# OvO1111/JointImageGeneration

Hardware: AMD Instinct MI355X
Metric: sampled voxels/sec @50 DDIM steps, 128^3 mask + 512^2x256 CT (higher is better)
Workload: dtype bf16; 1 GPU; C5 full GuideGen volume per GPU: CCDM 128^3 K=14 250 steps -> LDM 256 slices x (cond-encode + 50 DDIM @4x64x64 + AE decode 512^2); volumes_per_gpu=1, ccdm_steps=250, ddim_steps=50, slices=256, parallelism=replicas x1 (one volume per GPU, no collective), weights=random-init (seed recipe)

## Files before the change

include/guidegen_hip.h:

```cpp
#ifndef GUIDEGEN_HIP_H
#define GUIDEGEN_HIP_H

#include <stdint.h>

#ifdef __cplusplus
extern "C" {
#endif

typedef enum {
    GG_OK = 0,
    GG_ERR_BAD_SHAPE = -1,
    GG_ERR_BAD_DTYPE = -2,
    GG_ERR_UNSUPPORTED = -3,
    GG_ERR_WORKSPACE_TOO_SMALL = -4,
    GG_ERR_HIP = -5
} gg_status;

typedef enum { GG_BF16 = 0, GG_F32 = 1 } gg_dtype;

const char *gg_last_error(void);
int gg_version(void);

typedef struct {
    int32_t N, D, H, W;
// ... 29 lines not shown
    int32_t epilogue_geglu;
    int32_t pro_c_logical;
    const int64_t *pro_acc1;
    const int64_t *pro_acc2;
    const float *pro_gamma;
    const float *pro_beta;
    float pro_eps;
    int32_t skip_C1, skip_C2;
    int32_t reserved_tail;
    const void *skip_src1;
    const void *skip_src2;
    const void *skip_weight;
    const int32_t *post_xt;
    int32_t *post_labels_out;
    const float *post_scalars;
    const float *post_E;
    uint64_t post_philox_seed;
    const int64_t *post_philox_offset_dev;
    void *post_onehot_out;
    int64_t post_onehot_stride;
    int32_t post_draw;
    int32_t reserved_tail2;
    const uint64_t *post_philox_seeds;
    int64_t post_rows_per_sample;
} gg_conv_desc;

int64_t gg_conv_packed_weight_bytes(int32_t Cout, int32_t Cin_pad, int32_t ntaps);
int gg_conv_pack_weight(const float *w_f32, int32_t Cout, int32_t Cin, int32_t Cin_pad, int32_t ntaps,
                        void *packed_bf16, void *stream);
int64_t gg_conv_workspace_bytes(const gg_conv_desc *desc);
int gg_conv_fuses_prologue(const gg_conv_desc *desc);
int gg_conv_fuses_posterior(const gg_conv_desc *desc);
int gg_conv_runs_halo_tile(const gg_conv_desc *desc);
int gg_conv_emits_stats(const gg_conv_desc *desc);
int gg_conv_prologue_from_acc(const gg_conv_desc *desc);
int gg_conv_fuses_skip(const gg_conv_desc *desc);
int gg_conv_fuses_ddim(const gg_conv_desc *desc);
int gg_conv_forward(const gg_conv_desc *desc, void *stream);

int64_t gg_groupnorm_workspace_bytes(int32_t N, int64_t S, int32_t C);
int gg_groupnorm_stats(const void *src1, int32_t C1, const void *src2, int32_t C2, int32_t N, int64_t S,
                       int32_t C_logical, const float *gamma, const float *beta, float eps,
                       float *scale_out, float *shift_out, void *workspace, int64_t workspace_bytes, void *stream);
int gg_groupnorm_apply(const void *src1, int32_t C1, const void *src2, int32_t C2, int32_t N, int64_t S,
                       const float *scale, const float *shift, int32_t act, void *out, void *stream);
int gg_groupnorm_fused_supported(int64_t S, int32_t C1, int32_t C2, int32_t C_logical);
int gg_groupnorm_fused(const void *src1, int32_t C1, const void *src2, int32_t C2, int32_t N, int64_t S, int32_t C_logical,
                       const float *gamma, const float *beta, float eps, int32_t act, void *out, void *stream);
int gg_groupnorm_apply_acc(const void *src1, int32_t C1, const int64_t *acc1, const void *src2, int32_t C2, const int64_t *acc2,
                           int32_t N, int64_t S, int32_t C_logical, const float *gamma, const float *beta, float eps,
                           int32_t act, void *out, void *stream);

int gg_groupnorm_scale_shift_acc(const int64_t *acc1, int32_t stripes1, int32_t C1, const int64_t *acc2, int32_t stripes2, int32_t C2,
                                 int32_t N, int64_t S, int32_t C_logical, const float *gamma, const float *beta, float eps,
                                 float *scale_out, float *shift_out, void *stream);

int gg_resample2x(const void *src, int32_t dtype, int32_t N, int32_t D, int32_t H, int32_t W, int32_t C_pad, int32_t C_logical,
                  int32_t resample_d, int32_t mode, const float *scale, const float *shift, int32_t act, void *dst, void *stream);
int gg_film_fold(float *scale, float *shift, int32_t coef_stride, int32_t N, int32_t C, const float *film, int64_t film_stride, void *stream);

typedef struct {
    int32_t N, heads, head_dim;
    int32_t Tq, Tkv;
    int64_t ldq, hsq, ldk, hsk, ldv, hsv, ldo, hso;
    float scale;
    int32_t reserved;
// ... 157 lines not shown
```

jointimagegeneration_amd/_lib.py:

```python
from __future__ import annotations

import ctypes as C
import os

_HERE = os.path.dirname(os.path.abspath(__file__))
LIB_PATH = os.path.join(_HERE, "csrc", "libguidegen_hip.so")

GG_BF16, GG_F32 = 0, 1

vp, i32, i64, u64, f32 = C.c_void_p, C.c_int32, C.c_int64, C.c_uint64, C.c_float


class ConvDesc(C.Structure):
    _fields_ = [
        ("N", i32), ("D", i32), ("H", i32), ("W", i32),
        ("C1", i32), ("C2", i32), ("Cout", i32), ("Cout_pad", i32),
        ("kd", i32), ("kh", i32), ("kw", i32), ("stride", i32), ("pad", i32), ("upsample", i32),
        ("Do", i32), ("Ho", i32), ("Wo", i32), ("out_dtype", i32), ("prologue_act", i32), ("path_hint", i32),
        ("src1", vp), ("src2", vp), ("weight", vp), ("bias", vp), ("bias_stride", i64),
        ("residual", vp), ("out", vp), ("gn_scale", vp), ("gn_shift", vp), ("workspace", vp), ("workspace_bytes", i64), ("reserved_ptr", vp), ("gn_acc", vp),
        ("ddim_x", vp), ("ddim_scalars", vp), ("ddim_pred_x0", vp), ("ddim_unet_in", vp), ("ddim_unet_in_stride", i64),
        ("epilogue_geglu", i32), ("pro_c_logical", i32), ("pro_acc1", vp), ("pro_acc2", vp), ("pro_gamma", vp), ("pro_beta", vp),
        ("pro_eps", f32), ("skip_C1", i32), ("skip_C2", i32), ("reserved_tail", i32), ("skip_src1", vp), ("skip_src2", vp), ("skip_weight", vp),
        ("post_xt", vp), ("post_labels_out", vp), ("post_scalars", vp), ("post_E", vp), ("post_philox_seed", C.c_uint64),
        ("post_philox_offset_dev", vp), ("post_onehot_out", vp), ("post_onehot_stride", i64), ("post_draw", i32), ("reserved_tail2", i32),
        ("post_philox_seeds", vp), ("post_rows_per_sample", i64),
    ]


class AttentionDesc(C.Structure):
    _fields_ = [
        ("N", i32), ("heads", i32), ("head_dim", i32), ("Tq", i32), ("Tkv", i32),
        ("ldq", i64), ("hsq", i64), ("ldk", i64), ("hsk", i64), ("ldv", i64), ("hsv", i64), ("ldo", i64), ("hso", i64),
        ("scale", f32), ("reserved", i32),
        ("q", vp), ("k", vp), ("v", vp), ("out", vp), ("workspace", vp), ("workspace_bytes", i64),
    ]


SIGNATURES = {
    "gg_last_error": (C.c_char_p, []),
    "gg_version": (C.c_int, []),
    "gg_conv_packed_weight_bytes": (i64, [i32, i32, i32]),
    "gg_conv_pack_weight": (C.c_int, [vp, i32, i32, i32, i32, vp, vp]),
    "gg_conv_forward": (C.c_int, [C.POINTER(ConvDesc), vp]),
    "gg_conv_workspace_bytes": (i64, [C.POINTER(ConvDesc)]),
    "gg_conv_fuses_prologue": (C.c_int, [C.POINTER(ConvDesc)]),
    "gg_conv_runs_halo_tile": (C.c_int, [C.POINTER(ConvDesc)]),
    "gg_conv_emits_stats": (C.c_int, [C.POINTER(ConvDesc)]),
    "gg_conv_prologue_from_acc": (C.c_int, [C.POINTER(ConvDesc)]),
    "gg_conv_fuses_skip": (C.c_int, [C.POINTER(ConvDesc)]),
    "gg_conv_fuses_ddim": (C.c_int, [C.POINTER(ConvDesc)]),
    "gg_conv_fuses_posterior": (C.c_int, [C.POINTER(ConvDesc)]),
    "gg_groupnorm_workspace_bytes": (i64, [i32, i64, i32]),
    "gg_groupnorm_stats": (C.c_int, [vp, i32, vp, i32, i32, i64, i32, vp, vp, f32, vp, vp, vp, i64, vp]),
    "gg_groupnorm_apply": (C.c_int, [vp, i32, vp, i32, i32, i64, vp, vp, i32, vp, vp]),
    "gg_groupnorm_apply_acc": (C.c_int, [vp, i32, vp, vp, i32, vp, i32, i64, i32, vp, vp, f32, i32, vp, vp]),
    "gg_groupnorm_fused_supported": (C.c_int, [i64, i32, i32, i32]),
    "gg_groupnorm_fused": (C.c_int, [vp, i32, vp, i32, i32, i64, i32, vp, vp, f32, i32, vp, vp]),
    "gg_groupnorm_scale_shift_acc": (C.c_int, [vp, i32, i32, vp, i32, i32, i32, i64, i32, vp, vp, f32, vp, vp, vp]),
    "gg_attention_forward": (C.c_int, [C.POINTER(AttentionDesc), vp]),
    "gg_attention_workspace_bytes": (i64, [C.POINTER(AttentionDesc)]),
    "gg_attention_plan": (C.c_int, [C.POINTER(AttentionDesc), C.POINTER(i32)]),
    "gg_attention_forward_kvlen": (C.c_int, [C.POINTER(AttentionDesc), vp, vp]),
    "gg_layernorm": (C.c_int, [vp, i64, i32, vp, vp, f32, vp, vp]),
    "gg_geglu": (C.c_int, [vp, i64, i32, vp, vp]),
    "gg_add": (C.c_int, [vp, vp, i64, vp, vp]),
    "gg_linear_f32": (C.c_int, [vp, i32, i32, vp, vp, i32, i32, vp, i64, vp]),
    "gg_timestep_embedding": (C.c_int, [vp, i32, i32, f32, vp, vp]),
    "gg_nchw_f32_to_cl_bf16": (C.c_int, [vp, i32, i32, i64, vp, i32, i32, i32, vp]),
    "gg_cl_to_nchw_f32": (C.c_int, [vp, i32, i32, i32, i64, i32, vp, vp]),
    "gg_ccdm_posterior_sample": (C.c_int, [vp, i32, i32, vp, vp, u64, vp, i32, vp, i32, i64, vp, vp, vp, i32, vp]),
    "gg_ccdm_posterior_sample_seeds": (C.c_int, [vp, i32, i32, vp, vp, vp, i64, vp, i32, vp, i32, i64, vp, vp, vp, i32, vp]),
    "gg_ccdm_draw_tape": (C.c_int, [u64, vp, i64, vp, i32, i64, vp, vp, vp, vp]),
    "gg_labels_to_onehot": (C.c_int, [vp, i64, i32, vp, i32, vp]),
    "gg_ddim_step": (C.c_int, [vp, vp, i32, vp, vp, i64, i32, vp, vp, i32, vp]),
    "gg_minmax_normalise": (C.c_int, [vp, i64, vp, vp, vp]),
    "gg_ddpm_step": (C.c_int, [vp, vp, i32, vp, vp, i64, i32, vp, i32, vp]),
    "gg_inpaint_blend": (C.c_int, [vp, vp, vp, i32, vp, vp, i64, i32, vp, i32, vp]),
    "gg_ddpm_step_x0": (C.c_int, [vp, vp, i32, vp, vp, i32, i64, i32, vp, vp, i32, vp]),
    "gg_log_rows": (C.c_int, [vp, i32, i32, i64, vp, vp]),
    "gg_vq_nearest": (C.c_int, [vp, i32, vp, i32, i32, i64, vp, vp, i32, vp]),
# ... 72 lines not shown
```

jointimagegeneration_amd/csrc/gg_conv.h:

```cpp
#pragma once
#include "gg_common.h"

struct ConvParams {
    int N, D, H, W, C1, C2, Cout, Cout_pad;
    int kd, kh, kw, stride, pad, upsample;
    int Do, Ho, Wo, out_dtype, prologue_act;
    int path_hint;
    int nchunk1, nchunk, ntaps;
    long long M;
    long long bias_stride;
    const bf16_t *src1, *src2, *weight, *residual;
    const float *bias, *gn_scale, *gn_shift;
    void *out;
    float *ws;
    int splitk;
    long long *gn_acc;
    float *ddim_x, *ddim_pred_x0;
    const float *ddim_scalars;
    bf16_t *ddim_unet_in;
    long long ddim_unet_in_stride;
    unsigned mg_osp, mg_ohw, mg_wo;
    int epi_geglu;
    const long long *pro_acc1, *pro_acc2;
    const float *pro_gamma, *pro_beta;
    float pro_eps;
    int pro_clog;
    const bf16_t *skip_src1, *skip_src2, *skip_weight;
    int skip_C1, skip_C2;
    const int *post_xt;
    int *post_labels_out;
    const float *post_scalars, *post_E;
    unsigned long long post_seed;
    const long long *post_offset_dev;
    bf16_t *post_onehot_out;
    long long post_onehot_stride;
    int post_draw;
    const unsigned long long *post_seeds;
    long long post_rows_per_sample;
};

#define GG_BOX_HINT_GENERIC 10
#define GG_BOX_HINT_SPEC_ONLY 11
#define GG_HALO_HINT_BOX512 1
#define GG_HALO_HINT_BOX256 4
#define GG_HALO_HINT_BOX1024 6
#define GG_HALO_HINT_TEAM 7
#define GG_HALO_HINT_NO_TEAM 8

#define GG_ACC_SUM_SCALE 268435456.0f
#define GG_ACC_SQ_SCALE 1048576.0f
#ifndef GG_ACC_STRIPES
#define GG_ACC_STRIPES 1
#endif
#define GG_ACC_STRIPES_HALO 32

__device__ __forceinline__ int swz64(int row, int chunk) { return chunk ^ ((row >> 1) & 2); }


__device__ __forceinline__ float gg_row16_sum(float x)
{
    x += __builtin_bit_cast(float, __builtin_amdgcn_mov_dpp(__builtin_bit_cast(int, x), 0xB1, 0xF, 0xF, true));
    x += __builtin_bit_cast(float, __builtin_amdgcn_mov_dpp(__builtin_bit_cast(int, x), 0x4E, 0xF, 0xF, true));
    x += __builtin_bit_cast(float, __builtin_amdgcn_mov_dpp(__builtin_bit_cast(int, x), 0x141, 0xF, 0xF, true));
    x += __builtin_bit_cast(float, __builtin_amdgcn_mov_dpp(__builtin_bit_cast(int, x), 0x140, 0xF, 0xF, true));
    return x;
}
```

jointimagegeneration_amd/csrc/gg_conv.hip:

```cpp
#include "gg_norm.h"
#include <stdlib.h>

template <int NT, int PF, int PRO>
__global__ __launch_bounds__(256) void conv_gather_kernel(const ConvParams p)
{
    constexpr int BM = 128;
    constexpr int XBYTES = BM * 64;
    constexpr int WBYTES = NT * 32 * 64;
    constexpr int STAGE = XBYTES + WBYTES;
    constexpr int WITER = (NT * 128 + 255) / 256;
    __shared__ __attribute__((aligned(16))) char smem[2 * STAGE];

    const int tid = threadIdx.x;
    const int lane = tid & 63;
    const int wave = tid >> 6;
    const long long m0 = (long long)blockIdx.x * BM;
    const int g0 = blockIdx.y * NT;

    const int xq = tid & 3;
    int bn[2], bd[2], bh[2], bw[2];
    bool rv[2];
    const bf16_t *rb1[2], *rb2[2];
    const unsigned osp = (unsigned)(p.Do * p.Ho * p.Wo);
    const unsigned ohw = (unsigned)(p.Ho * p.Wo);
// ... 182 lines not shown
                bf16x4 ob;
#pragma unroll
                for (int j = 0; j < 4; ++j) {
                    const float ge = 0.5f * g[j] * (1.0f + erff(g[j] * 0.70710678118654752f));
                    ob[j] = (bf16_t)((oc + j < inner) ? v[j] * ge : 0.f);
                }
                *reinterpret_cast<bf16x4 *>((bf16_t *)p.out + m * ostride + oc) = ob;
            }
        }
        return;
    }
    f32x4 bv[2][2 * NT];
    bf16x4 resv[2][2 * NT];
#pragma unroll
    for (int pt = 0; pt < 2; ++pt) {
        const long long m = m0 + wave * 32 + pt * 16 + fr;
        const long long mc = m < p.M ? m : p.M - 1;
        const int n = (int)((unsigned)mc / osp);
        const float *brow = p.bias ? p.bias + (long long)n * p.bias_stride : nullptr;
#pragma unroll
        for (int ct = 0; ct < 2 * NT; ++ct) {
            const int co = (g0 * 32) + ct * 16 + fq * 4;
            bv[pt][ct] = brow ? *reinterpret_cast<const f32x4 *>(brow + co) : f32x4{0.f, 0.f, 0.f, 0.f};
            if (p.residual) resv[pt][ct] = *reinterpret_cast<const bf16x4 *>(p.residual + mc * p.Cout_pad + co);
        }
    }
#pragma unroll
    for (int pt = 0; pt < 2; ++pt) {
        long long m = m0 + wave * 32 + pt * 16 + fr;
        if (m >= p.M) continue;
#pragma unroll
        for (int ct = 0; ct < 2 * NT; ++ct) {
            int co = (g0 * 32) + ct * 16 + fq * 4;
            f32x4 v = acc[pt][ct];
            if (p.bias) v += bv[pt][ct];
            long long o = m * p.Cout_pad + co;
            if (p.residual) {
                const bf16x4 r = resv[pt][ct];
#pragma unroll
                for (int j = 0; j < 4; ++j) v[j] += (float)r[j];
            }
#pragma unroll
            for (int j = 0; j < 4; ++j)
                if (co + j >= p.Cout) v[j] = 0.f;
            if (p.out_dtype == GG_F32) {
                *reinterpret_cast<f32x4 *>((float *)p.out + o) = v;
            } else {
                bf16x4 ob;
#pragma unroll
                for (int j = 0; j < 4; ++j) ob[j] = (bf16_t)v[j];
                *reinterpret_cast<bf16x4 *>((bf16_t *)p.out + o) = ob;
            }
        }
    }
}

template <int PRO>
__global__ __launch_bounds__(256) void conv_gather5_kernel(const ConvParams p)
{
    constexpr int BM = 64, CPS = 5;
    constexpr int XT = BM * 64, WT = 32 * 64;
    constexpr int STAGE = CPS * (XT + WT);
    constexpr int GNMAX = 2560;
    __shared__ __attribute__((aligned(16))) char smem[2 * STAGE + (PRO ? 2 * GNMAX * 4 : 0)];
    const int tid = threadIdx.x, lane = tid & 63;
    const int wave = __builtin_amdgcn_readfirstlane(tid >> 6);
    const int fr = lane & 15, fq = lane >> 4;
    const long long m0 = (long long)blockIdx.x * BM;
    const int g0 = blockIdx.y;
    float *gns = reinterpret_cast<float *>(smem + 2 * STAGE);

    const int xrow = tid >> 2, xq = tid & 3;
    const unsigned osp = (unsigned)(p.Do * p.Ho * p.Wo), ohw = (unsigned)(p.Ho * p.Wo);
    bool rv;
    int bd, bh, bw;
    const bf16_t *rb1, *rb2;
    {
        long long m = m0 + xrow;
        rv = m < p.M;
        unsigned mu = rv ? (unsigned)m : 0u;
        unsigned n = (unsigned)gg_fastdiv(mu, (int)osp, p.mg_osp), r = mu - n * osp;
        unsigned od = (unsigned)gg_fastdiv(r, (int)ohw, p.mg_ohw);
        r -= od * ohw;
        unsigned oh = (unsigned)gg_fastdiv(r, p.Wo, p.mg_wo), ow = r - oh * (unsigned)p.Wo;
// ... 405 lines not shown
    p.post_seeds = (const unsigned long long *)d->post_philox_seeds; p.post_rows_per_sample = d->post_rows_per_sample;
    p.mg_osp = gg_magic_u32(p.M, d->Do * d->Ho * d->Wo); p.mg_ohw = gg_magic_u32(p.M, d->Ho * d->Wo); p.mg_wo = gg_magic_u32(p.M, d->Wo);
}

static bool halo_try_dry(const ConvParams &p) { return gg_conv_halo_try(p, (hipStream_t)-1) == GG_OK; }
static bool box_try_dry(const ConvParams &p) { return gg_conv_box_try(p, (hipStream_t)-1) == GG_OK; }
static bool desc_channels_ok(const gg_conv_desc *d) { return d && d->C1 > 0 && d->C1 % 32 == 0 && d->C2 % 32 == 0 && d->Cout_pad % 32 == 0; }

static int take_splitk_workspace(const gg_conv_desc *d, ConvParams &p, int splitk)
{
    if (splitk > 1) {
        const long long need = (long long)splitk * p.M * p.Cout_pad * 4;
        if (!d->workspace || d->workspace_bytes < need)
            GG_FAIL(GG_ERR_WORKSPACE_TOO_SMALL, "conv: split-K needs %lld workspace bytes (gg_conv_workspace_bytes), got %lld", need, (long long)d->workspace_bytes);
        p.ws = (float *)d->workspace;
    }
    p.splitk = splitk;
    return GG_OK;
}

extern "C" int gg_conv_runs_halo_tile(const gg_conv_desc *d)
{
    if (!desc_channels_ok(d) || d->epilogue_geglu) return 0;
    ConvParams p;
    fill_params(d, p);
    return halo_try_dry(p) ? 1 : 0;
}

extern "C" int gg_conv_fuses_prologue(const gg_conv_desc *d)
{
    if (!desc_channels_ok(d) || d->epilogue_geglu) return 0;
    ConvParams p;
    fill_params(d, p);
    if (halo_try_dry(p)) return (GG_HALO_SEPARATE_NORM && d->path_hint == 0 && gg_conv_halo_prefers_separate_norm(p)) ? 0 : 1;
    if (box_try_dry(p)) return gg_conv_box_fuses_prologue(p) ? 1 : 0;
    return 0;
}

bool gg_conv_box_emits_stats(const ConvParams &p);
bool gg_conv_box_prologue_from_acc(const ConvParams &p);
bool gg_conv_halo_fuses_posterior(const ConvParams &p);

extern "C" int gg_conv_fuses_posterior(const gg_conv_desc *d)
{
    if (!desc_channels_ok(d) || d->epilogue_geglu || d->residual || d->out_dtype != GG_F32 || d->gn_acc ||
        d->ddim_x || d->skip_C1) return 0;
    ConvParams p;
    fill_params(d, p);
    return gg_conv_halo_fuses_posterior(p) ? 1 : 0;
}

extern "C" int gg_conv_prologue_from_acc(const gg_conv_desc *d)
{
    if (!desc_channels_ok(d) || d->epilogue_geglu || !d->prologue_act) return 0;
    if (d->pro_c_logical <= 0 || d->pro_c_logical % 32 || d->pro_c_logical > d->C1 + d->C2 || (d->C2 && d->pro_c_logical < d->C1)) return 0;
    ConvParams p;
    fill_params(d, p);
    if (halo_try_dry(p)) return 0;
    return box_try_dry(p) && gg_conv_box_prologue_from_acc(p) ? 1 : 0;
}

extern "C" int gg_conv_fuses_skip(const gg_conv_desc *d)
{
    if (!desc_channels_ok(d) || d->epilogue_geglu || d->skip_C1 <= 0 || d->skip_C1 % 32 || d->skip_C2 % 32 ||
        d->skip_C2 < 0 || d->residual || d->ddim_x)
        return 0;
    ConvParams p;
    fill_params(d, p);
    if (halo_try_dry(p)) return 0;
    return box_try_dry(p) ? 1 : 0;
}

extern "C" int gg_conv_fuses_ddim(const gg_conv_desc *d)
{
    if (!desc_channels_ok(d) || d->out_dtype != GG_F32 || d->Cout != 4 || d->residual) return 0;
    ConvParams p;
    fill_params(d, p);
    if (halo_try_dry(p)) return 0;
    return box_try_dry(p) ? 1 : 0;
}


extern "C" int gg_conv_emits_stats(const gg_conv_desc *d)
{
    if (!desc_channels_ok(d) || d->out_dtype != GG_BF16 || d->epilogue_geglu) return 0;
    ConvParams p;
    fill_params(d, p);
    if (halo_try_dry(p)) return GG_ACC_STRIPES_HALO;
    if (box_try_dry(p)) return gg_conv_box_emits_stats(p) ? GG_ACC_STRIPES : 0;
    if (gg_conv_tiny_plan(p.M, p.Cout_pad, p.ntaps * p.nchunk, p.prologue_act)) return 0;
    const long long osp = (long long)d->Do * d->Ho * d->Wo;
    return (plan_gather5(p.M, p.C1, p.C2, p.Cout_pad, p.ntaps) == 1 && osp % 64 == 0) ? GG_ACC_STRIPES : 0;
}

#ifdef GG_EXP_WPREFETCH
__global__ __launch_bounds__(256) void exp_wprefetch_kernel(const u32x4 *w, long long n16, unsigned *sink)
{
    unsigned a = 0;
    if (n16 <= (3 << 20) / 16 * 1) {
        for (long long i = (long long)(blockIdx.x >> 3) * 256 + threadIdx.x; i < n16; i += 32 * 256) { const u32x4 v = w[i]; a ^= v[0] ^ v[1] ^ v[2] ^ v[3]; }
    } else
    for (long long i = (long long)blockIdx.x * 256 + threadIdx.x; i < n16; i += 256 * 256) { const u32x4 v = w[i]; a ^= v[0] ^ v[1] ^ v[2] ^ v[3]; }
    if (a == 0x12345679u) sink[0] = a;
}
#endif
extern "C" int gg_conv_forward(const gg_conv_desc *d, void *stream_)
{
    hipStream_t stream = (hipStream_t)stream_;
    if (!d) GG_FAIL(GG_ERR_BAD_SHAPE, "conv: null desc");
    if (d->C1 <= 0 || d->C1 % 32 || d->C2 % 32 || d->C2 < 0) GG_FAIL(GG_ERR_BAD_SHAPE, "conv: C1/C2 must be multiples of 32 (got %d, %d)", d->C1, d->C2);
    if (d->Cout_pad % 32 || d->Cout > d->Cout_pad || d->Cout <= 0) GG_FAIL(GG_ERR_BAD_SHAPE, "conv: bad Cout/Cout_pad %d/%d", d->Cout, d->Cout_pad);
    auto okk = [](int k) { return k == 1 || k == 3; };
    if (!okk(d->kd) || !okk(d->kh) || !okk(d->kw)) GG_FAIL(GG_ERR_UNSUPPORTED, "conv: kernel extent must be 1 or 3");
    if (d->stride != 1 && d->stride != 2) GG_FAIL(GG_ERR_UNSUPPORTED, "conv: stride must be 1 or 2");
    if (d->upsample && d->stride != 1) GG_FAIL(GG_ERR_UNSUPPORTED, "conv: upsample with stride");
    if (d->out_dtype != GG_BF16 && d->out_dtype != GG_F32) GG_FAIL(GG_ERR_BAD_DTYPE, "conv: out dtype");
    if (!d->src1 || !d->weight || (!d->out && !d->post_xt) || (d->C2 && !d->src2)) GG_FAIL(GG_ERR_BAD_SHAPE, "conv: null pointer");
    if (d->post_xt) {
        if (!gg_conv_fuses_posterior(d)) GG_FAIL(GG_ERR_UNSUPPORTED, "conv: this shape cannot run the fused CCDM reverse step (gg_conv_fuses_posterior)");
        if (!d->post_labels_out || !d->post_scalars) GG_FAIL(GG_ERR_BAD_SHAPE, "conv: fused CCDM reverse step needs labels_out and scalars");
        if (d->post_onehot_out && (d->post_onehot_stride < d->Cout || (d->post_onehot_stride & 1) || ((uintptr_t)d->post_onehot_out & 3)))
            GG_FAIL(GG_ERR_BAD_SHAPE, "conv: fused CCDM reverse step: one-hot rows must be 4-byte aligned (even stride >= K)");
        if (d->post_philox_seeds && d->post_rows_per_sample != (int64_t)d->Do * d->Ho * d->Wo)
            GG_FAIL(GG_ERR_BAD_SHAPE, "conv: fused CCDM reverse step: post_rows_per_sample %lld must be Do*Ho*Wo = %lld",
                    (long long)d->post_rows_per_sample, (long long)d->Do * d->Ho * d->Wo);
// ... 25 lines not shown
    if (p.M >= (1LL << 31) || (long long)d->D * d->H * d->W * (d->C1 > d->C2 ? d->C1 : d->C2) >= (1LL << 31))
        GG_FAIL(GG_ERR_UNSUPPORTED, "conv: tensor too large for 32-bit in-sample offsets");

    if (d->epilogue_geglu) {
        if (d->kd != 1 || d->kh != 1 || d->kw != 1 || d->stride != 1 || d->upsample || d->residual || d->out_dtype != GG_BF16 || d->gn_acc ||
            d->ddim_x || d->Cout % 32 || d->bias_stride)
            GG_FAIL(GG_ERR_UNSUPPORTED, "conv: the GEGLU epilogue needs a 1x1 conv, bf16 output, Cout = 2*inner with inner %% 16 == 0, a shared bias, no residual / gn_acc / ddim");
        return launch_gather_nt(plan_gather(p.M, p.Cout_pad, p.ntaps * p.nchunk).NT, p, stream);
    }
#ifdef GG_EXP_WPREFETCH
    {
        const long long wbytes = (long long)(p.Cout_pad / 32) * p.ntaps * p.nchunk * 2048;
        hipLaunchKernelGGL(exp_wprefetch_kernel, dim3(256), dim3(256), 0, stream, (const u32x4 *)p.weight, wbytes >> 4, (unsigned *)d->out);
    }
#endif
#ifdef GG_H3_STAMPS
    if (d->path_hint == GG_HALO_HINT_TEAM && d->workspace) p.ws = (float *)d->workspace;
#endif
    int rc = gg_conv_halo_try(p, stream);
#ifdef GG_H3_STAMPS
    p.ws = nullptr;
#endif
    if (rc != GG_ERR_UNSUPPORTED) return rc;
    if (d->post_xt) GG_FAIL(GG_ERR_UNSUPPORTED, "conv: the halo-tile kernel did not take this shape, and no other kernel runs the fused CCDM reverse step");
#ifdef GG_BOX_STAMPS
    if (d->path_hint == 98) p.ws = (float *)d->workspace;
#endif
    rc = gg_conv_box_try(p, stream);
#ifdef GG_BOX_STAMPS
    p.ws = nullptr;
#endif
    if (rc != GG_ERR_UNSUPPORTED) return rc;

    if (int tsk = gg_conv_tiny_plan(p.M, p.Cout_pad, p.ntaps * p.nchunk, p.prologue_act)) {
        if ((rc = take_splitk_workspace(d, p, tsk)) != GG_OK) return rc;
        rc = gg_conv_tiny_launch(p, stream);
        if (rc != GG_OK || tsk == 1) return rc;
        return launch_splitk_reduce(p, stream, false);
    }

    if (int s5 = plan_gather5(p.M, p.C1, p.C2, p.Cout_pad, p.ntaps)) {
        if ((rc = take_splitk_workspace(d, p, s5)) != GG_OK) return rc;
        dim3 grid((unsigned)((p.M + 63) / 64), (unsigned)(p.Cout_pad / 32), (unsigned)s5);
        if (p.prologue_act && (((long long)p.Do * p.Ho * p.Wo) % 64 || p.C1 + p.C2 > 2560))
            GG_FAIL(GG_ERR_UNSUPPORTED, "conv: fused prologue on the 160-step kernel needs Do*Ho*Wo %% 64 == 0 and C <= 2560");
        if (p.prologue_act) hipLaunchKernelGGL(conv_gather5_kernel<1>, grid, dim3(256), 0, stream, p);
        else hipLaunchKernelGGL(conv_gather5_kernel<0>, grid, dim3(256), 0, stream, p);
        GG_CHECK_LAUNCH();
        return s5 > 1 ? launch_splitk_reduce(p, stream, true) : GG_OK;
    }

    GatherPlan pl = plan_gather(p.M, p.Cout_pad, p.ntaps * p.nchunk);
    if ((rc = take_splitk_workspace(d, p, pl.splitk)) != GG_OK) return rc;
    return launch_gather_nt(pl.NT, p, stream);
}
```

jointimagegeneration_amd/csrc/gg_conv_halo.hip:

```cpp
#include <atomic>
#include "gg_norm.h"
#include "gg_posterior.h"
#include <stdlib.h>
#ifndef GG_HALO_G3
#define GG_HALO_G3 1
#endif
#ifndef GG_HALO_G3_2D
#define GG_HALO_G3_2D 1
#endif
#ifndef GG_HALO_2D_HB1
#define GG_HALO_2D_HB1 1
#endif
#ifndef GG_HALO_G3_HB1
#define GG_HALO_G3_HB1 1
#endif
#ifndef GG_HALO_TSTORE
#define GG_HALO_TSTORE 1
#endif
#ifndef GG_HALO_W16_2D
#define GG_HALO_W16_2D 1
#endif
struct HaloBox { int TD, TH, TW; };
constexpr HaloBox halo_box(bool d3, int hb) { return d3 ? HaloBox{hb == 2 ? 8 : 4, hb == 1 ? 4 : 8, 16} : HaloBox{1, hb == 1 ? 16 : 32, 16}; }

// ... 434 lines not shown
}

constexpr int halo_key(int d3, int nt, int up, int hb, int post) { return (((d3 * 8 + nt) * 2 + up) * 4 + hb) * 2 + post; }
static int halo_dispatch(const ConvParams &p, const HaloPlan &pl, hipStream_t stream)
{
#define GG_HALO_CASE(D3, NT, UP, HB, POST) case halo_key(D3, NT, UP, HB, POST): return launch_halo<D3, NT, UP, HB, POST>(p, pl, stream);
    switch (halo_key(pl.d3, pl.NT, pl.up, pl.HB, pl.post)) {
        GG_HALO_CASE(1, 2, 0, 2, 0) GG_HALO_CASE(1, 1, 0, 2, 1) GG_HALO_CASE(1, 1, 0, 2, 0)
        GG_HALO_CASE(1, 2, 1, 1, 0) GG_HALO_CASE(1, 2, 0, 1, 0) GG_HALO_CASE(1, 1, 1, 1, 0) GG_HALO_CASE(1, 1, 0, 1, 0)
        GG_HALO_CASE(1, 4, 1, 0, 0) GG_HALO_CASE(1, 3, 1, 0, 0) GG_HALO_CASE(1, 2, 1, 0, 0) GG_HALO_CASE(1, 1, 1, 0, 0)
        GG_HALO_CASE(1, 4, 0, 0, 0) GG_HALO_CASE(1, 3, 0, 0, 0) GG_HALO_CASE(1, 2, 0, 0, 0) GG_HALO_CASE(1, 1, 0, 0, 0)
        GG_HALO_CASE(0, 4, 1, 1, 0) GG_HALO_CASE(0, 4, 0, 1, 0) GG_HALO_CASE(0, 3, 1, 1, 0) GG_HALO_CASE(0, 3, 0, 1, 0)
        GG_HALO_CASE(0, 4, 1, 0, 0) GG_HALO_CASE(0, 3, 1, 0, 0) GG_HALO_CASE(0, 2, 1, 0, 0) GG_HALO_CASE(0, 1, 1, 0, 0)
        GG_HALO_CASE(0, 4, 0, 0, 0) GG_HALO_CASE(0, 3, 0, 0, 0) GG_HALO_CASE(0, 2, 0, 0, 0) GG_HALO_CASE(0, 1, 0, 0, 0)
        default: return GG_ERR_UNSUPPORTED;
    }
#undef GG_HALO_CASE
}

int gg_conv_halo3_try(const ConvParams &p, hipStream_t stream);

static int halo_pick_nt(bool d3, int G, long long tiles)
{
    for (int want : {!d3 ? 128 : 256, 128})
        for (int cand : {4, 3, 2, 1})
            if (G % cand == 0 && tiles * (G / cand) >= want) return cand;
    return 1;
}

static HaloPlan halo_plan(const ConvParams &p)
{
    HaloPlan pl{};
    const int hint = p.path_hint;
    const bool prod = hint == 0 || hint == GG_HALO_HINT_NO_TEAM;
    pl.d3 = (p.kd == 3); pl.up = p.upsample ? 1 : 0; pl.post = p.post_xt ? 1 : 0;
    const HaloBox b0 = halo_box(pl.d3, 0);
    const int G = p.Cout_pad / 32;
    const long long tiles = (long long)p.N * (p.Do / b0.TD) * (p.Ho / b0.TH) * (p.Wo / b0.TW);
    pl.NT = halo_pick_nt(pl.d3, G, tiles);
    pl.blocks = tiles * (G / pl.NT);
    if (pl.d3 && pl.NT <= 2 && !pl.up && (p.Do % 8) == 0 && (hint == GG_HALO_HINT_BOX1024 || (prod && pl.blocks >= 512))) pl.HB = 2;
    else if (pl.d3 && pl.NT <= 2 && (hint == GG_HALO_HINT_BOX256 || (prod && pl.blocks <= 256))) pl.HB = 1;
    else if (!pl.d3 && GG_HALO_2D_HB1 && pl.NT >= 3 && (hint == GG_HALO_HINT_BOX256 || (prod && pl.blocks < 224))) pl.HB = 1;
    const HaloBox b = halo_box(pl.d3, pl.HB);
    pl.tiles_d = p.Do / b.TD; pl.tiles_h = p.Ho / b.TH; pl.tiles_w = p.Wo / b.TW;
    pl.family = p.kh == 3 && p.kw == 3 && (p.kd == 3 || p.kd == 1) && p.stride == 1 && p.pad == 1 && (pl.d3 || p.D == 1);
    const bool gate = hint != GG_HALO_HINT_BOX512 && hint != GG_HALO_HINT_BOX256 && hint != GG_HALO_HINT_BOX1024 && hint != GG_HALO_HINT_TEAM;
    pl.ok = pl.family && !(p.Wo % b0.TW || p.Ho % b0.TH || p.Do % b0.TD) && !(gate && pl.blocks < ((pl.d3 || pl.NT > 1) ? 128 : 256));
    return pl;
}

bool gg_conv_halo_prefers_separate_norm(const ConvParams &p)
{
    const HaloPlan pl = halo_plan(p);
    const int groups = p.Cout_pad / 32 / pl.NT;
    return groups >= 3 || (groups == 2 && pl.NT == 4);
}

bool gg_conv_halo_fuses_posterior(const ConvParams &p)
{
    if (p.Cout > 16 || p.Cout_pad != 32 || p.out_dtype != GG_F32 || p.residual || p.gn_acc) return false;
    const HaloPlan pl = halo_plan(p);
    return pl.ok && pl.HB == 2;
}

int gg_conv_halo_try(const ConvParams &p, hipStream_t stream)
{
// ... 14 lines not shown
```

jointimagegeneration_amd/ops.py:

```python
from __future__ import annotations

import ctypes as C
from dataclasses import dataclass
from typing import Optional, Sequence, Tuple

import torch

from . import _lib
from ._lib import GG_BF16, GG_F32, AttentionDesc, ConvDesc, check


def _stream() -> int:
    return torch.cuda.current_stream().cuda_stream


def _ptr(t: Optional[torch.Tensor]) -> Optional[int]:
    return None if t is None else t.data_ptr()


def require_gpu(t: torch.Tensor, what: str) -> None:
    if not t.is_cuda:
        raise RuntimeError(f"{what}: tensor is on {t.device}; the GuideGen engine runs on MI355X only "
                           "(no CPU fallback; the CPU restatement lives in oracle/ and is test infrastructure)")


FP32 = False


class fp32_validation:
    def __enter__(self):
        global FP32
        self.prev, FP32 = FP32, True
        return self

    def __exit__(self, *exc):
        global FP32
        FP32 = self.prev
        return False


def is_f32(t) -> bool:
    return t.dtype == torch.float32


PATH_HINT = 0
def weights_token(module) -> Tuple[int, int, int]:
    n = v = a = 0
    for p in module.parameters():
        n += 1
        v += p._version
        a += p.data_ptr()
    return n, v, a


def invalidate_caches(module) -> None:
    with torch.no_grad():
        for p in module.parameters():
            p.add_(0)


def capture_graph(fn) -> "torch.cuda.CUDAGraph":
    import gc
    g = torch.cuda.CUDAGraph()
    gc.collect()
    was_enabled = gc.isenabled()
    gc.disable()
    try:
        with torch.cuda.graph(g):
            fn()
    finally:
        if was_enabled:
            gc.enable()
    return g


def pad32(c: int) -> int:
    return (c + 31) // 32 * 32

# ... 1304 lines not shown
```

Baseline: 815,500 voxels/s.

## Add persistent LDS-resident-weight tiled kernel for large 1x1 convolutions

Adds a new 1x1 convolution kernel that keeps the whole packed weight in LDS and runs persistent waves over 32-row tiles. Each wave prefetches the next activation tile into registers while it computes the current one with MFMA, then stages outputs through LDS so global stores are coalesced. It is dispatched ahead of the tiny/gather paths for large M with bf16 output and no residual or prologue, and a new GATHER hint keeps the old path reachable. The aim is to avoid re-reading weights and to get better memory coalescing on the big 1x1 convs in the autoencoder decoder. In exchange it brings in new kernel instances, high LDS usage that limits occupancy, and a shared epilogue helper.

```diff
diff --git a/include/guidegen_hip.h b/include/guidegen_hip.h
--- a/include/guidegen_hip.h
+++ b/include/guidegen_hip.h
@@ -85,6 +85,7 @@
 int gg_conv_fuses_prologue(const gg_conv_desc *desc);
 int gg_conv_fuses_posterior(const gg_conv_desc *desc);
 int gg_conv_runs_halo_tile(const gg_conv_desc *desc);
+int gg_conv_runs_tile(const gg_conv_desc *desc);
 int gg_conv_emits_stats(const gg_conv_desc *desc);
 int gg_conv_prologue_from_acc(const gg_conv_desc *desc);
 int gg_conv_fuses_skip(const gg_conv_desc *desc);
diff --git a/jointimagegeneration_amd/_lib.py b/jointimagegeneration_amd/_lib.py
--- a/jointimagegeneration_amd/_lib.py
+++ b/jointimagegeneration_amd/_lib.py
@@ -47,6 +47,7 @@
     "gg_conv_fuses_prologue": (C.c_int, [C.POINTER(ConvDesc)]),
     "gg_conv_runs_halo_tile": (C.c_int, [C.POINTER(ConvDesc)]),
     "gg_conv_emits_stats": (C.c_int, [C.POINTER(ConvDesc)]),
+    "gg_conv_runs_tile": (C.c_int, [C.POINTER(ConvDesc)]),
     "gg_conv_prologue_from_acc": (C.c_int, [C.POINTER(ConvDesc)]),
     "gg_conv_fuses_skip": (C.c_int, [C.POINTER(ConvDesc)]),
     "gg_conv_fuses_ddim": (C.c_int, [C.POINTER(ConvDesc)]),
diff --git a/jointimagegeneration_amd/csrc/gg_conv.h b/jointimagegeneration_amd/csrc/gg_conv.h
--- a/jointimagegeneration_amd/csrc/gg_conv.h
+++ b/jointimagegeneration_amd/csrc/gg_conv.h
@@ -46,6 +46,8 @@
 #define GG_HALO_HINT_BOX1024 6
 #define GG_HALO_HINT_TEAM 7
 #define GG_HALO_HINT_NO_TEAM 8
+#define GG_CONV_HINT_GATHER 12
+static inline bool gg_hint_is_production(int hint) { return hint == 0 || hint == GG_CONV_HINT_GATHER; }
 
 #define GG_ACC_SUM_SCALE 268435456.0f
 #define GG_ACC_SQ_SCALE 1048576.0f
@@ -65,3 +67,27 @@
     x += __builtin_bit_cast(float, __builtin_amdgcn_mov_dpp(__builtin_bit_cast(int, x), 0x140, 0xF, 0xF, true));
     return x;
 }
+
+__device__ __forceinline__ f32x4 gg_conv_epi_value(f32x4 acc, bool has_bias, f32x4 bv, bool has_res, bf16x4 res, int co, int Cout)
+{
+    f32x4 v = acc;
+    if (has_bias) v += bv;
+    if (has_res) {
+#pragma unroll
+        for (int j = 0; j < 4; ++j) v[j] += (float)res[j];
+    }
+#pragma unroll
+    for (int j = 0; j < 4; ++j)
+        if (co + j >= Cout) v[j] = 0.f;
+    return v;
+}
+__device__ __forceinline__ bf16x4 gg_conv_epi_bf16(f32x4 v)
+{
+    bf16x4 ob;
+#pragma unroll
+    for (int j = 0; j < 4; ++j) ob[j] = (bf16_t)v[j];
+    return ob;
+}
+
+int gg_conv_tile_try(const ConvParams &p, hipStream_t stream);
+int gg_conv_tile_family(const ConvParams &p);
diff --git a/jointimagegeneration_amd/csrc/gg_conv.hip b/jointimagegeneration_amd/csrc/gg_conv.hip
--- a/jointimagegeneration_amd/csrc/gg_conv.hip
+++ b/jointimagegeneration_amd/csrc/gg_conv.hip
@@ -238,24 +238,12 @@
 #pragma unroll
         for (int ct = 0; ct < 2 * NT; ++ct) {
             int co = (g0 * 32) + ct * 16 + fq * 4;
-            f32x4 v = acc[pt][ct];
-            if (p.bias) v += bv[pt][ct];
+            const f32x4 v = gg_conv_epi_value(acc[pt][ct], p.bias != nullptr, bv[pt][ct], p.residual != nullptr, resv[pt][ct], co, p.Cout);
             long long o = m * p.Cout_pad + co;
-            if (p.residual) {
-                const bf16x4 r = resv[pt][ct];
-#pragma unroll
-                for (int j = 0; j < 4; ++j) v[j] += (float)r[j];
-            }
-#pragma unroll
-            for (int j = 0; j < 4; ++j)
-                if (co + j >= p.Cout) v[j] = 0.f;
             if (p.out_dtype == GG_F32) {
                 *reinterpret_cast<f32x4 *>((float *)p.out + o) = v;
             } else {
-                bf16x4 ob;
-#pragma unroll
-                for (int j = 0; j < 4; ++j) ob[j] = (bf16_t)v[j];
-                *reinterpret_cast<bf16x4 *>((bf16_t *)p.out + o) = ob;
+                *reinterpret_cast<bf16x4 *>((bf16_t *)p.out + o) = gg_conv_epi_bf16(v);
             }
         }
     }
@@ -727,7 +715,7 @@
     if (!desc_channels_ok(d) || d->epilogue_geglu) return 0;
     ConvParams p;
     fill_params(d, p);
-    if (halo_try_dry(p)) return (GG_HALO_SEPARATE_NORM && d->path_hint == 0 && gg_conv_halo_prefers_separate_norm(p)) ? 0 : 1;
+    if (halo_try_dry(p)) return (GG_HALO_SEPARATE_NORM && gg_hint_is_production(d->path_hint) && gg_conv_halo_prefers_separate_norm(p)) ? 0 : 1;
     if (box_try_dry(p)) return gg_conv_box_fuses_prologue(p) ? 1 : 0;
     return 0;
 }
@@ -786,6 +774,15 @@
     if (gg_conv_tiny_plan(p.M, p.Cout_pad, p.ntaps * p.nchunk, p.prologue_act)) return 0;
     const long long osp = (long long)d->Do * d->Ho * d->Wo;
     return (plan_gather5(p.M, p.C1, p.C2, p.Cout_pad, p.ntaps) == 1 && osp % 64 == 0) ? GG_ACC_STRIPES : 0;
+}
+
+extern "C" int gg_conv_runs_tile(const gg_conv_desc *d)
+{
+    if (!desc_channels_ok(d) || d->epilogue_geglu || d->skip_C1 || d->ddim_x || d->post_xt) return 0;
+    ConvParams p;
+    fill_params(d, p);
+    if (halo_try_dry(p) || box_try_dry(p)) return 0;
+    return gg_conv_tile_family(p);
 }
 
 #ifdef GG_EXP_WPREFETCH
@@ -877,6 +874,9 @@
 #endif
     if (rc != GG_ERR_UNSUPPORTED) return rc;
 
+    rc = gg_conv_tile_try(p, stream);
+    if (rc != GG_ERR_UNSUPPORTED) return rc;
+
     if (int tsk = gg_conv_tiny_plan(p.M, p.Cout_pad, p.ntaps * p.nchunk, p.prologue_act)) {
         if ((rc = take_splitk_workspace(d, p, tsk)) != GG_OK) return rc;
         rc = gg_conv_tiny_launch(p, stream);
diff --git a/jointimagegeneration_amd/csrc/gg_conv_halo.hip b/jointimagegeneration_amd/csrc/gg_conv_halo.hip
--- a/jointimagegeneration_amd/csrc/gg_conv_halo.hip
+++ b/jointimagegeneration_amd/csrc/gg_conv_halo.hip
@@ -490,7 +490,7 @@
 {
     HaloPlan pl{};
     const int hint = p.path_hint;
-    const bool prod = hint == 0 || hint == GG_HALO_HINT_NO_TEAM;
+    const bool prod = gg_hint_is_production(hint) || hint == GG_HALO_HINT_NO_TEAM;
     pl.d3 = (p.kd == 3); pl.up = p.upsample ? 1 : 0; pl.post = p.post_xt ? 1 : 0;
     const HaloBox b0 = halo_box(pl.d3, 0);
     const int G = p.Cout_pad / 32;
diff --git a/jointimagegeneration_amd/csrc/gg_conv_tile.hip b/jointimagegeneration_amd/csrc/gg_conv_tile.hip
--- /dev/null
+++ b/jointimagegeneration_amd/csrc/gg_conv_tile.hip
@@ -0,0 +1,207 @@
+#include "gg_conv.h"
+#include <atomic>
+
+#ifndef GG_TILE_CONV
+#define GG_TILE_CONV 1
+#endif
+
+#define GG_TILE_MIN_M 262144
+
+template <int CT, int NCH>
+struct TileGeom {
+    static constexpr int NWAVE = 4, ROWS = 32;
+    static constexpr int COUT = CT * 16;
+    static constexpr int WBYTES = (CT / 2) * NCH * 2048;
+    static constexpr int XBYTES = NCH * ROWS * 64;
+    static constexpr int ORS = COUT * 2 + 16;
+    static constexpr int OBYTES = ROWS * ORS;
+    static constexpr int STAGE = XBYTES > OBYTES ? XBYTES : OBYTES;
+    static constexpr int S0 = WBYTES;
+    static constexpr int LDSB = S0 + NWAVE * STAGE;
+    static constexpr int XLOADS = 2 * NCH;
+    static constexpr int OSTORES = CT;
+    static_assert(CT % 2 == 0 && COUT <= 128, "whole 32-cout groups of the packed weight");
+    static_assert(S0 % 16 == 0 && STAGE % 16 == 0 && ORS % 16 == 0, "16-byte LDS accesses stay aligned");
+    static_assert((NCH - 1) * ROWS * 64 + (ROWS - 1) * 64 + 3 * 16 + 16 <= STAGE, "activation tile inside the stage");
+    static_assert((ROWS - 1) * ORS + ((CT - 1) * 16 + 3 * 4) * 2 + 8 <= STAGE, "output tile inside the stage");
+    static_assert((ROWS - 1) * ORS + (COUT / 8 - 1) * 16 + 16 <= STAGE, "output pieces inside the stage");
+    static_assert(((CT / 2 - 1) * NCH + NCH - 1) * 2048 + 31 * 64 + 3 * 16 + 16 <= WBYTES, "weight fragments inside the image");
+    static_assert(ROWS * NCH * 4 == XLOADS * 64 && ROWS * (COUT / 8) == OSTORES * 64, "pieces divide evenly over the lanes");
+    static_assert(LDSB <= 160 * 1024, "fits the CU's LDS");
+    static constexpr int PER_CU = 2 * LDSB <= 160 * 1024 ? 2 : 1;
+};
+
+__device__ __forceinline__ void tile_wave_lds_fence()
+{
+    asm volatile("" ::: "memory");
+    __builtin_amdgcn_wave_barrier();
+}
+
+template <int CT, int NCH>
+__global__ __launch_bounds__(256, (TileGeom<CT, NCH>::PER_CU)) void conv_tile1x1_kernel(const ConvParams p)
+{
+    using G = TileGeom<CT, NCH>;
+    extern __shared__ __attribute__((aligned(16))) char smem[];
+    const int tid = threadIdx.x, lane = tid & 63;
+    const int wave = __builtin_amdgcn_readfirstlane(tid >> 6);
+    const int fr = lane & 15, fq = lane >> 4;
+
+    for (int i = tid; i < G::WBYTES / 16; i += 256)
+        *reinterpret_cast<u32x4 *>(smem + i * 16) = *reinterpret_cast<const u32x4 *>(p.weight + (long long)i * 8);
+    __syncthreads();
+
+    char *st = smem + G::S0 + wave * G::STAGE;
+    const long long ntiles = (p.M + G::ROWS - 1) / G::ROWS;
+    const long long tstep = (long long)gridDim.x * G::NWAVE;
+    const int n1 = 2 * p.nchunk1;
+    const int sh1 = 31 - __builtin_clz((unsigned)p.C1 >> 3);
+    const int sh2 = p.C2 ? 31 - __builtin_clz((unsigned)p.C2 >> 3) : 0;
+    const unsigned osp = (unsigned)(p.Do * p.Ho * p.Wo);
+
+    u32x4 xr[G::XLOADS];
+    auto load_tile = [&](long long t) {
+        const long long m0 = t * G::ROWS;
+        const int valid = (int)(p.M - m0 < G::ROWS ? p.M - m0 : G::ROWS);
+        const bf16_t *b1 = p.src1 + m0 * p.C1;
+        const bf16_t *b2 = p.src2 ? p.src2 + m0 * p.C2 : nullptr;
+#pragma unroll
+        for (int j = 0; j < G::XLOADS; ++j) {
+            const bool first = j < n1;
+            const int i = lane + 64 * (first ? j : j - n1);
+            const int row = i >> (first ? sh1 : sh2);
+            u32x4 v = {0u, 0u, 0u, 0u};
+            if (row < valid) v = *reinterpret_cast<const u32x4 *>((first ? b1 : b2) + i * 8);
+            xr[j] = v;
+        }
+    };
+    auto stage_tile = [&]() {
+#pragma unroll
+        for (int j = 0; j < G::XLOADS; ++j) {
+            const bool first = j < n1;
+            const int i = lane + 64 * (first ? j : j - n1);
+            const int sh = first ? sh1 : sh2;
+            const int row = i >> sh, pc = i & ((1 << sh) - 1);
+            const int chunk = (first ? 0 : p.nchunk1) + (pc >> 2);
+            *reinterpret_cast<u32x4 *>(st + chunk * (G::ROWS * 64) + row * 64 + swz64(row, pc & 3) * 16) = xr[j];
+        }
+    };
+
+    long long t = (long long)blockIdx.x * G::NWAVE + wave;
+    if (t < ntiles) load_tile(t);
+    for (; t < ntiles; t += tstep) {
+        const long long m0 = t * G::ROWS;
+        const int valid = (int)(p.M - m0 < G::ROWS ? p.M - m0 : G::ROWS);
+        stage_tile();
+        tile_wave_lds_fence();
+        f32x4 bv[2][CT];
+#pragma unroll
+        for (int pt = 0; pt < 2; ++pt) {
+            const long long m = m0 + pt * 16 + fr;
+            const long long mc = m < p.M ? m : p.M - 1;
+            const float *brow = p.bias ? p.bias + (long long)((unsigned)mc / osp) * p.bias_stride : nullptr;
+#pragma unroll
+            for (int ct = 0; ct < CT; ++ct)
+                bv[pt][ct] = brow ? *reinterpret_cast<const f32x4 *>(brow + ct * 16 + fq * 4) : f32x4{0.f, 0.f, 0.f, 0.f};
+        }
+        if (t + tstep < ntiles) load_tile(t + tstep);
+
+        f32x4 acc[2][CT];
+#pragma unroll
+        for (int pt = 0; pt < 2; ++pt)
+#pragma unroll
+            for (int ct = 0; ct < CT; ++ct) acc[pt][ct] = f32x4{0.f, 0.f, 0.f, 0.f};
+#pragma unroll
+        for (int c = 0; c < NCH; ++c) {
+            bf16x8 xf[2];
+#pragma unroll
+            for (int pt = 0; pt < 2; ++pt) {
+                const int r = pt * 16 + fr;
+                xf[pt] = *reinterpret_cast<const bf16x8 *>(st + c * (G::ROWS * 64) + r * 64 + swz64(r, fq) * 16);
+            }
+#pragma unroll
+            for (int ct = 0; ct < CT; ++ct) {
+                const int r = (ct & 1) * 16 + fr;
+                const bf16x8 wf = *reinterpret_cast<const bf16x8 *>(smem + ((ct >> 1) * NCH + c) * 2048 + r * 64 + swz64(r, fq) * 16);
+#pragma unroll
+                for (int pt = 0; pt < 2; ++pt)
+                    acc[pt][ct] = __builtin_amdgcn_mfma_f32_16x16x32_bf16(wf, xf[pt], acc[pt][ct], 0, 0, 0);
+            }
+        }
+        tile_wave_lds_fence();
+
+#pragma unroll
+        for (int pt = 0; pt < 2; ++pt) {
+            const int r = pt * 16 + fr;
+#pragma unroll
+            for (int ct = 0; ct < CT; ++ct) {
+                const int co = ct * 16 + fq * 4;
+                const f32x4 v = gg_conv_epi_value(acc[pt][ct], p.bias != nullptr, bv[pt][ct], false, bf16x4{}, co, p.Cout);
+                *reinterpret_cast<bf16x4 *>(st + r * G::ORS + co * 2) = gg_conv_epi_bf16(v);
+            }
+        }
+        tile_wave_lds_fence();
+        bf16_t *ob = (bf16_t *)p.out + m0 * G::COUT;
+#pragma unroll
+        for (int j = 0; j < G::OSTORES; ++j) {
+            const int i = lane + 64 * j;
+            const int row = i / (G::COUT / 8), pc = i % (G::COUT / 8);
+            const u32x4 v = *reinterpret_cast<const u32x4 *>(st + row * G::ORS + pc * 16);
+            if (row < valid) *reinterpret_cast<u32x4 *>(ob + i * 8) = v;
+        }
+        tile_wave_lds_fence();
+    }
+}
+
+static bool pow2(int v) { return v > 0 && (v & (v - 1)) == 0; }
+
+static bool tile_instantiated(int CT, int NCH)
+{
+    return (CT == 4 && (NCH == 4 || NCH == 6)) || (CT == 8 && (NCH == 2 || NCH == 6 || NCH == 8));
+}
+
+int gg_conv_tile_family(const ConvParams &p)
+{
+    if (!GG_TILE_CONV || p.path_hint == GG_CONV_HINT_GATHER) return 0;
+    if (p.kd != 1 || p.kh != 1 || p.kw != 1 || p.stride != 1 || p.upsample) return 0;
+    if (p.Do != p.D || p.Ho != p.H || p.Wo != p.W) return 0;
+    if (p.prologue_act || p.residual || p.out_dtype != GG_BF16 || p.epi_geglu || p.post_xt || p.ddim_x || p.skip_C1) return 0;
+    if (p.Cout_pad != 64 && p.Cout_pad != 128) return 0;
+    if (!pow2(p.C1) || p.C1 < 32 || (p.C2 && (!pow2(p.C2) || p.C2 < 32))) return 0;
+    if (!tile_instantiated(p.Cout_pad / 16, p.nchunk)) return 0;
+    if (p.M < GG_TILE_MIN_M) return 0;
+    return 1;
+}
+
+template <int CT, int NCH>
+static int launch_tile1x1(const ConvParams &p, hipStream_t stream)
+{
+    using G = TileGeom<CT, NCH>;
+    int dev = 0, cus = 0;
+    if (hipGetDevice(&dev) != hipSuccess || hipDeviceGetAttribute(&cus, hipDeviceAttributeMultiprocessorCount, dev) != hipSuccess) return GG_ERR_HIP;
+    static std::atomic<unsigned long long> attr_mask{0};
+    const unsigned long long dev_bit = 1ull << (dev & 63);
+    if (!(attr_mask.load(std::memory_order_acquire) & dev_bit)) {
+        if (hipFuncSetAttribute((const void *)conv_tile1x1_kernel<CT, NCH>, hipFuncAttributeMaxDynamicSharedMemorySize, G::LDSB) != hipSuccess) return GG_ERR_UNSUPPORTED;
+        attr_mask.fetch_or(dev_bit, std::memory_order_release);
+    }
+    const int per_cu = G::PER_CU;
+    const long long ntiles = (p.M + G::ROWS - 1) / G::ROWS;
+    long long blocks = (ntiles + G::NWAVE - 1) / G::NWAVE;
+    if (blocks > (long long)cus * per_cu) blocks = (long long)cus * per_cu;
+    hipLaunchKernelGGL((conv_tile1x1_kernel<CT, NCH>), dim3((unsigned)blocks), dim3(256), G::LDSB, stream, p);
+    GG_CHECK_LAUNCH();
+    return GG_OK;
+}
+
+int gg_conv_tile_try(const ConvParams &p, hipStream_t stream)
+{
+    if (gg_conv_tile_family(p) != 1) return GG_ERR_UNSUPPORTED;
+    if (stream == (hipStream_t)-1) return GG_OK;
+    const int CT = p.Cout_pad / 16;
+    if (CT == 4 && p.nchunk == 4) return launch_tile1x1<4, 4>(p, stream);
+    if (CT == 4 && p.nchunk == 6) return launch_tile1x1<4, 6>(p, stream);
+    if (CT == 8 && p.nchunk == 2) return launch_tile1x1<8, 2>(p, stream);
+    if (CT == 8 && p.nchunk == 6) return launch_tile1x1<8, 6>(p, stream);
+    if (CT == 8 && p.nchunk == 8) return launch_tile1x1<8, 8>(p, stream);
+    return GG_ERR_UNSUPPORTED;
+}
diff --git a/jointimagegeneration_amd/ops.py b/jointimagegeneration_amd/ops.py
--- a/jointimagegeneration_amd/ops.py
+++ b/jointimagegeneration_amd/ops.py
@@ -44,6 +44,7 @@
 
 
 PATH_HINT = 0
+HINT_GATHER = 12
 def weights_token(module) -> Tuple[int, int, int]:
     n = v = a = 0
     for p in module.parameters():
```

Result: faster. 823,900 voxels/s (median of 6 runs) (+1.0%).
